# hzxie/Stereo-3D-Reconstruction

Measured on NVIDIA B200. Metric: stereo pairs/sec Stereo2Voxel fwd, higher is better.
Workload: dtype bf16

## Files before the change

### include/s3d.h

```cpp
#ifndef S3D_H_
#define S3D_H_

#include <stdint.h>

#ifdef __cplusplus
extern "C" {
#endif

#define S3D_OK                0
#define S3D_ERR_INVALID      -1
#define S3D_ERR_CUDA         -2
#define S3D_ERR_UNSUPPORTED  -3

#define S3D_DTYPE_F32   0
#define S3D_DTYPE_BF16  1
#define S3D_DTYPE_BF16X2 2

#define S3D_ACT_NONE     0
#define S3D_ACT_RELU     1
#define S3D_ACT_LEAKY    2
#define S3D_ACT_SIGMOID  3
#define S3D_ACT_TANH     4

#define S3D_MAX_TAPS 64

typedef struct S3dConvParams {
  int32_t N, iD, iH, iW, Cin;
  int32_t oD, oH, oW, Cout;
  int32_t sz, sy, sx;
  int32_t ntaps, n_classes;
  int8_t  dz[S3D_MAX_TAPS], dy[S3D_MAX_TAPS], dx[S3D_MAX_TAPS];
  int64_t osN, osD, osH, osW;
  int64_t osC;
  int64_t os_lo;
  int32_t omz, omy, omx;
  int32_t cout_store;
  int32_t in_dtype, out_dtype;
  int32_t act;  float act_param;
  int32_t tw, th, td, tn;
  int32_t bn;
  const float* proj_w;
  int32_t proj_channel, proj_act;
  const void* w_nstack;
  int32_t dz_nref, dz_c, dz_e, dz_pairs;
  const int32_t* dz_sched;
  long long* dz_planes;
} S3dConvParams;

const char* s3d_version(void);
const char* s3d_last_error(void);
int s3d_device_check(int dev);
int s3d_set_knob(const char* name, int value);
int s3d_get_knob(const char* name);

int s3d_conv_igemm(const S3dConvParams* p, const void* in, const void* w, const float* bias,
                   const void* residual, void* out, void* stream);
int s3d_conv_direct(const S3dConvParams* p, const void* in, const void* w, const float* bias,
                    const void* residual, void* out, void* stream);

int s3d_conv2d_halo(const void* in, const void* w, const float* bias, const void* residual, void* out, int nimg, int h, int wd,
                    int cin, int cout, int64_t osN, int64_t osH, int64_t osW, int relu, void* stream);

int s3d_pack_image(const float* img, const float* disp, float disp_scale, void* out,
                   int B, int H, int W, int Cpad, int out_dtype, void* stream);

int s3d_pack_image_u8(const uint8_t* img, const float* disp, float disp_scale, float img_scale, void* out,
                      int B, int H, int W, int Cpad, int out_dtype, void* stream);

int s3d_conv_first(const void* img, int img_u8, const float* disp, float disp_scale, const void* w, const float* bias,
                   void* out, int B, int H, int W, int cin, int cin_pad, int cout_pad, int dtype, int act,
                   float act_param, void* stream);

int s3d_conv_concat_volume(const S3dConvParams* p, const void* feat, int feat_pitch, int feat_pad, const float* bias,
                           void* out, void* stream);
int s3d_conv_concat_volume_ro(const S3dConvParams* p, const void* feat, int feat_pitch, int feat_pad, const void* w_refonce,
                              const float* bias, void* out, void* stream);
int s3d_concat_gonce_assemble(const float* maps_l, const float* maps_r, const float* edge_l, const float* edge_r,
                              const float* bias, void* out, int B, int D, int h, int w, int map_w, int out_dtype, void* stream);
int s3d_map_conv(const void* in, const void* w, float* out, int nimg, int h, int in_w, int ow, int off, int ntx, int cout,
                 int dtype, void* stream);
int s3d_cost_volume_concat(const void* feat, void* vol, int B, int h, int w, int C, int D,
                           int dtype, void* stream);
int s3d_soft_argmin(const float* cost, float* disp, int N, int D, int h, int w, float sign,
                    void* stream);


int s3d_tap_gather_soft_argmin(const float* taps, float* disp, float* disp_std_q, float* cost_out, int N, int D, int h, int w,
                               int tap_stride, float sign, void* stream);
int s3d_cls_soft_argmin(const void* x, const void* w_taps, float* disp, float* disp_std_q, int N, int D, int h, int w, int C,
                        float sign, void* stream);
int64_t s3d_conv_cls_workspace_bytes(int N, int D, int h, int w);
int s3d_conv_cls_soft_argmin(const S3dConvParams* p, const void* in, const float* bias, const void* w_taps, void* workspace,
                             float* disp, float* disp_std_q, float sign, void* stream);
int s3d_corr_soft_argmin(const void* feat, float* disp, float* disp_std_q, float* cost_out, int B, int h, int w,
                         int C, int c_real, int D, int dtype, void* stream);
int s3d_upsample_disp(const float* disp_q, float* disp, int N, int h, int w, int H, int W,
                      float scale, void* stream);
int s3d_upsample_disp_eval(const float* disp_q, float* disp, int B, int h, int w, int H, int W, float scale,
                           const float* gt, const float* thresholds, int T, float max_gt, long long* disp_stats,
                           uint8_t* lr_mask, float lr_thresh, long long* lr_stats,
                           const float* disp_std_q, float* disp_std, const float* unc_thresh, int K, long long* unc_stats,
                           void* stream);

int s3d_latent_to_vox(const void* x, void* out, int N, int H, int W, int C, int L, int dtype,
                      void* stream);
int s3d_avg_pool(const void* x, void* out, int N, int H, int W, int C, int L, int dtype,
                 void* stream);
int s3d_depth_to_space(const void* in, void* out, const float* proj_w, int proj_act, int N, int d, int h, int w,
                       int Cpad, int dtype, void* stream);
int s3d_split_tf32(const float* x, float* hi, float* lo, int64_t n, void* stream);
int s3d_split_bf16(const float* x, void* out, int64_t npix, int C, void* stream);
// ... 28 lines not shown
```

### stereo_3d_reconstruction_b200/csrc/concat_gonce.cu

```cuda
#include "common.cuh"

namespace s3d {
namespace {

constexpr int kMaps = 6 * 64;
constexpr int kEdge = 4 * 64;

__device__ __forceinline__ void add8(float (&v)[8], const float* __restrict__ p) {
  const float4 a = __ldg(reinterpret_cast<const float4*>(p)), b = __ldg(reinterpret_cast<const float4*>(p) + 1);
  v[0] += a.x;  v[1] += a.y;  v[2] += a.z;  v[3] += a.w;  v[4] += b.x;  v[5] += b.y;  v[6] += b.z;  v[7] += b.w;
}

template <bool kSplit>
__global__ void __launch_bounds__(256)
gonce_assemble_kernel(const float* __restrict__ maps_l, const float* __restrict__ maps_r, const float* __restrict__ edge_l,
                      const float* __restrict__ edge_r, const float* __restrict__ bias, __nv_bfloat16* __restrict__ out,
                      int B, int D, int h, int w, int mw) {
  const int x = blockIdx.x * 32 + (threadIdx.x >> 3), co = (threadIdx.x & 7) * 8;
  const int y = blockIdx.y, n = blockIdx.z;
  if (x >= w) return;
  const bool left_ref = n < B;
  const int b = left_ref ? n : n - B;
  const float* pm = (left_ref ? maps_l : maps_r) + (((int64_t)b * h + y) * mw + (x + 2)) * kMaps + co;
  const float* gm = (left_ref ? maps_r : maps_l) + ((int64_t)b * h + y) * mw * kMaps + 3 * 64 + co;
  const bool edge = x == (left_ref ? w - 1 : 0);
  const float* em = (left_ref ? edge_r : edge_l) + ((int64_t)b * h + y) * D * kEdge + co;
  float base[8];
  {
    const float4 b0 = __ldg(reinterpret_cast<const float4*>(bias + co)), b1 = __ldg(reinterpret_cast<const float4*>(bias + co) + 1);
    base[0] = b0.x;  base[1] = b0.y;  base[2] = b0.z;  base[3] = b0.w;  base[4] = b1.x;  base[5] = b1.y;  base[6] = b1.z;  base[7] = b1.w;
    add8(base, pm);
  }
  constexpr int kCo = kSplit ? 128 : 64;
  __nv_bfloat16* op = out + ((((int64_t)n * D) * h + y) * w + x) * kCo + co;
  const int64_t plane = (int64_t)h * w * kCo;
#pragma unroll 4
  for (int d = 0; d < D; ++d) {
    float v[8];
#pragma unroll
    for (int i = 0; i < 8; ++i) v[i] = base[i];
    const int col = (left_ref ? x - d : x + d) + 2;
    const bool in = col >= 0 && col < mw;
    if (in) add8(v, gm + (int64_t)col * kMaps);
    if (d == 0)     { add8(v, pm + 64);   if (in) add8(v, gm + (int64_t)col * kMaps + 64); }
    if (d == D - 1) { add8(v, pm + 128);  if (in) add8(v, gm + (int64_t)col * kMaps + 128); }
    if (edge) {
      const float* e = em + (int64_t)(left_ref ? D - 1 - d : d) * kEdge;
      add8(v, e);
      if (d == 0) add8(v, e + 64);
      if (d == D - 1) add8(v, e + 128);
    }
    uint32_t oh[4], ol[4];
#pragma unroll
    for (int i = 0; i < 4; ++i) {
      const float a0 = fmax_nan(v[2 * i], 0.f), a1 = fmax_nan(v[2 * i + 1], 0.f);
      __nv_bfloat162 t = __floats2bfloat162_rn(a0, a1);
      oh[i] = *reinterpret_cast<uint32_t*>(&t);
      if constexpr (kSplit) {
        const float2 hf = __bfloat1622float2(t);
        __nv_bfloat162 l = __floats2bfloat162_rn(a0 - hf.x, a1 - hf.y);
        ol[i] = *reinterpret_cast<uint32_t*>(&l);
      }
    }
    const uint4 o = make_uint4(oh[0], oh[1], oh[2], oh[3]);
    __stcs(reinterpret_cast<uint4*>(op + d * plane), o);
    if constexpr (kSplit) __stcs(reinterpret_cast<uint4*>(op + d * plane + 64), make_uint4(ol[0], ol[1], ol[2], ol[3]));
  }
}

}
}

extern "C" int s3d_concat_gonce_assemble(const float* maps_l, const float* maps_r, const float* edge_l, const float* edge_r,
                                         const float* bias, void* out, int B, int D, int h, int w, int map_w, int out_dtype,
                                         void* stream) {
  using namespace s3d;
  if (!maps_l || !maps_r || !edge_l || !edge_r || !bias || !out) { set_error("concat_gonce_assemble: null argument"); return S3D_ERR_INVALID; }
  S3D_CHECK_ARG(B > 0 && D >= 2 && h > 0 && w > 0 && map_w == w + 4, "concat_gonce_assemble: B=%d D=%d h=%d w=%d map_w=%d (needs D >= 2, map_w = w + 4)", B, D, h, w, map_w);
  S3D_CHECK_ARG(((reinterpret_cast<uintptr_t>(maps_l) | reinterpret_cast<uintptr_t>(maps_r) | reinterpret_cast<uintptr_t>(edge_l) |
                  reinterpret_cast<uintptr_t>(edge_r) | reinterpret_cast<uintptr_t>(bias) | reinterpret_cast<uintptr_t>(out)) & 15) == 0,
                "concat_gonce_assemble: pointers must be 16-byte aligned");
  S3D_CHECK_ARG(h <= 65535 && 2 * B <= 65535, "concat_gonce_assemble: grid too large");
  S3D_CHECK_ARG(out_dtype == S3D_DTYPE_BF16 || out_dtype == S3D_DTYPE_BF16X2, "concat_gonce_assemble: out_dtype %d", out_dtype);
  dim3 grid(ceil_div(w, 32), h, 2 * B);
  if (out_dtype == S3D_DTYPE_BF16X2)
    gonce_assemble_kernel<true><<<grid, 256, 0, static_cast<cudaStream_t>(stream)>>>(maps_l, maps_r, edge_l, edge_r, bias,
                                                                                     static_cast<__nv_bfloat16*>(out), B, D, h, w, map_w);
  else
    gonce_assemble_kernel<false><<<grid, 256, 0, static_cast<cudaStream_t>(stream)>>>(maps_l, maps_r, edge_l, edge_r, bias,
                                                                                      static_cast<__nv_bfloat16*>(out), B, D, h, w, map_w);
  S3D_LAUNCH_CHECK();
  return S3D_OK;
}
```

### stereo_3d_reconstruction_b200/csrc/conv_scatter.cu

```cuda
#include "conv_scatter.cuh"

namespace s3d {
using namespace scatter;

bool conv_scatter_eligible(const S3dConvParams* p) {
  const int esz = p->in_dtype == S3D_DTYPE_F32 ? 4 : 2;
  const bool split = p->in_dtype == S3D_DTYPE_BF16X2;
  if (!p->w_nstack || knobs().no_scatter) return false;
  if (split && (p->out_dtype != S3D_DTYPE_BF16X2 || p->Cin > 64 || (p->Cout != 16 && p->Cout != 32 && p->Cout != 64) ||
                p->cout_store != p->Cout)) return false;
  if (!split && p->out_dtype == S3D_DTYPE_BF16X2) return false;
  if (!plane_scatter_layer(*p)) return false;
  const int cin_bytes = (split ? 2 : 1) * p->Cin * esz;
  if (split && cin_bytes == 32) return false;
  if (cin_bytes != 32 && cin_bytes != 64 && cin_bytes != 128 && cin_bytes != 256) return false;
  if (p->Cout > 64 || p->Cout % 16 != 0) return false;
  return true;
}

int conv_scatter_launch(const S3dConvParams* p_in, const void* in, const float* bias, const void* residual, void* out,
                        cudaStream_t stream) {
  const S3dConvParams& p = *p_in;
  const bool tf32 = p.in_dtype == S3D_DTYPE_F32;
  const bool split = p.in_dtype == S3D_DTYPE_BF16X2;
  const int esz = tf32 ? 4 : 2;
  const int cin_phys = split ? 2 * p.Cin : p.Cin;
  S3D_CHECK_ARG(p.cout_store >= 1 && p.cout_store <= p.Cout, "scatter: cout_store");
  ScArgs a;
  memset(&a, 0, sizeof(a));
  a.p = p;  a.bias = bias;  a.residual = residual;  a.out = out;
  a.split = split ? 1 : 0;
  a.os_lo = p.os_lo ? p.os_lo : (int64_t)p.Cout;
  const int nchunks = cin_phys * esz == 256 ? 2 : 1;
  int64_t total = plane_geometry(a, cin_phys * esz / nchunks, cin_phys / nchunks, nchunks);
  a.cp = p.Cout;
  a.tps = spec_tps(a.row_bytes, a.cp);
  if (knobs().scatter_tps3 && a.tps == 9) a.tps = 3;
  S3D_CHECK_ARG(total > 0 && total < (1ll << 31), "scatter: column count out of range");
  {
    const int sms = num_sms();
    int nz = knobs().scatter_zsplit > 0 ? knobs().scatter_zsplit : (knobs().scatter_zsplit < 0 ? 1 : (int)(sms / total));
    if (nz > p.oD / 4) nz = p.oD / 4;
    if (nz > 1) {
      a.zc = ceil_div(p.oD, nz);
      a.nz = ceil_div(p.oD, a.zc);
      a.dl = a.zc + 2;
      if (a.nz > 1) total *= a.nz; else { a.nz = 1; a.zc = p.oD; a.dl = p.oD; }
    }
  }
  int grid = num_sms();
  a.pair = ((3 * a.cp / 2) % 8 == 0 && total >= 2 && grid >= 2 && !knobs().scatter_no_pair) ? 1 : 0;
  const bool fast_ok = coalesced_store_ok(p, bias, out, residual, p.out_dtype == S3D_DTYPE_F32 ? 4 : 2) &&
                       (split || !knobs().scatter_no_transpose);
  const bool two = fast_ok && a.pair && !tf32 && !split && a.nchunks == 1 && p.out_dtype == S3D_DTYPE_BF16 && residual == nullptr &&
                   spec_kernel(a.row_bytes, a.cp, false, p.act == S3D_ACT_RELU, true) != nullptr && total > grid &&
                   !knobs().scatter_generic && !knobs().scatter_one_cta && !knobs().scatter_tps3 && !knobs().scatter_ring;
  if (two) grid *= 2;
  grid = deal_columns(a, total, grid);
  const bool dz = p.dz_nref > 0 && !tf32 && !split && a.nz == 1 && !knobs().no_dz_skip;
  if (dz) S3D_CHECK_ARG(p.N == 2 * p.dz_nref && p.dz_c >= 0 && p.dz_e >= 0, "scatter: constant-region descriptor");
  if (!dz) a.p.dz_nref = 0;
  if (!dz || !a.pair) a.p.dz_sched = nullptr;
  if (a.p.dz_sched) {
    S3D_CHECK_ARG(p.dz_pairs >= 1, "scatter: dz_pairs");
    grid = 2 * p.dz_pairs;
  }
  const int w_rows = a.pair ? 3 * a.cp / 2 : 3 * a.cp;
  a.w_tx = a.tps * w_rows * a.row_bytes;
  a.w_bytes = align1024(a.w_tx);
  const int budget = two ? 110 * 1024 : 227 * 1024 - 1024 - 512;
  int ring = (budget - 4 * a.w_bytes) / a.slot_bytes;
  if (ring > kMaxRing) ring = kMaxRing;
  if (ring < 2) ring = 2;
  if (a.row_bytes == 128 && ring > (a.pair && a.nchunks == 1 ? 3 : 2)) ring = a.pair && a.nchunks == 1 ? 3 : 2;
  if (const int r = knobs().scatter_ring) { if (r >= 2 && r <= kMaxRing) ring = r; }
  a.ring = ring;
  a.w_stages = (budget - a.ring * a.slot_bytes) / a.w_bytes;
  if (a.w_stages > kMaxW) a.w_stages = kMaxW;
  S3D_CHECK_ARG(a.w_stages >= 2, "scatter: not enough shared memory for the weight ring");
  a.idesc = ptx::make_instr_desc(tf32 ? 2 : 1, a.pair ? 256 : 128, 3 * a.cp);
  a.res_direct = !knobs().scatter_res_transpose;
  a.fast_store = fast_ok;
  if (split) {
    S3D_CHECK_ARG(a.fast_store && (a.os_lo * 2) % 16 == 0 && a.os_lo >= p.Cout,
                  "scatter (split operands): needs a bias, a none / ReLU / LeakyReLU activation and 16-byte aligned out / residual / strides");
    a.res_direct = 1;
  }

  const CUtensorMapSwizzle sw = a.row_bytes == 128 ? CU_TENSOR_MAP_SWIZZLE_128B
                              : a.row_bytes == 64 ? CU_TENSOR_MAP_SWIZZLE_64B : CU_TENSOR_MAP_SWIZZLE_32B;
  CUtensorMap map_x, map_w;
  cuuint32_t box[5] = {(cuuint32_t)a.kc, kHX, kHY, 1, 1};
// ... 8 lines not shown
                  p.osW == 64 && p.osH == (int64_t)p.oW * 64 && p.osD == (int64_t)p.oH * p.osH && p.osN == (int64_t)p.oD * p.osD &&
                  !knobs().scatter_no_rm && !knobs().scatter_generic;
  if (rm) {
    const int extra = kResBytes + 32 * 128;
    a.w_stages = (budget - a.ring * a.slot_bytes - extra) / a.w_bytes;
    if (a.w_stages > kMaxW) a.w_stages = kMaxW;
    S3D_CHECK_ARG(a.w_stages >= 3, "scatter: not enough shared memory for the residual stage");
    CUtensorMap map_r;
    cuuint32_t rbox[5] = {64, kTX, kTY, 1, 1};
    rc = encode_act_map(&map_r, residual, 2, false, 64, p.oW, p.oH, p.oD, p.N, rbox, estr, CU_TENSOR_MAP_SWIZZLE_128B);
    if (rc != S3D_OK) return rc;
    a.residual = nullptr;
    const int smem_rm = a.ring * a.slot_bytes + a.w_stages * a.w_bytes + extra + 1024;
    return launch_plane_scatter(rm_kernel(p.act == S3D_ACT_RELU), grid, smem_rm, a.pair, stream, map_x, map_w, map_r, a);
  }

  const int smem_bytes = a.ring * a.slot_bytes + a.w_stages * a.w_bytes + 1024;
  KernFn kern = a.pair ? (tf32 ? conv_scatter_kernel<true, true> : conv_scatter_kernel<false, true>)
                       : (tf32 ? conv_scatter_kernel<true, false> : conv_scatter_kernel<false, false>);
  if (split) {
    const bool lean = a.pair && a.tps == spec_tps(a.row_bytes, a.cp) && !knobs().scatter_generic;
    kern = split_kernel(lean, a.pair != 0, cin_phys * esz, a.cp, residual != nullptr, p.act == S3D_ACT_RELU);
  }
  else if (a.pair && !tf32 && a.nchunks == 1 && p.out_dtype == S3D_DTYPE_BF16 && a.fast_store && a.tps == spec_tps(a.row_bytes, a.cp) &&
      !knobs().scatter_generic) {
    const bool relu = p.act == S3D_ACT_RELU;
    if (KernFn k = spec_kernel(a.row_bytes, a.cp, residual != nullptr, relu, two && a.fast_store)) kern = k;
    else if (two) { set_error("scatter: the two-CTA kernel needs the coalesced store path"); return S3D_ERR_INVALID; }
  }
  return launch_plane_scatter(kern, grid, smem_bytes, a.pair, stream, map_x, map_w, a);
}

}
```

### stereo_3d_reconstruction_b200/layers.py

```python
import ctypes
import os
import itertools

import torch

from . import lib as _lib

PAD = 16


def pad_to(c, m=PAD):
    return (c + m - 1) // m * m


def torch_dtype(code):
    return torch.float32 if code == _lib.DTYPE_F32 else torch.bfloat16


def is_split(code):
    return code == _lib.DTYPE_BF16X2


def cmult(code):
    return 2 if code == _lib.DTYPE_BF16X2 else 1
# ... 77 lines not shown
    return xr + c + 2


def dz_jump(zs, D, e):
    ze = D - 2 - e
    return (ze - zs) // 3 * 3 if ze - zs >= 3 else 0


def dz_march(zs, J, D):
    out, p = [], 0
    while p < D:
        out.append(p)
        p = p + 1 + J if p == zs + 1 else p + 1
    return out


def dz_schedule(N, nref, oH, oW, D, c, e, npairs):
    total = scatter_columns(N, oH, oW)
    first = [dz_first(k, N, nref, oH, oW, c) for k in range(total)]
    cols = sorted(range(total), key=lambda k: (first[k], k))
    items = [(cols[i], cols[i + 1] if i + 1 < total else total) for i in range(0, total, 2)]
    cost = [D - dz_jump(max(first[a], first[b] if b < total else 0), D, e) for a, b in items]
    load, lists = [0] * npairs, [[] for _ in range(npairs)]
    for i in sorted(range(len(items)), key=lambda i: (-cost[i], i)):
        q = min(range(npairs), key=lambda q: (load[q], q))
        load[q] += cost[i]
        lists[q].append(items[i])
    offs, ent = [0], []
    for lst in lists:
        offs.append(offs[-1] + len(lst))
        for a, b in lst:
            ent += [a, b]
    return offs + ent, load


class PackedConv:

    def __init__(self, w_rows, bias, taps, stride, out_mult, cin, cout, act, act_param, dtype_code, device,
                 ksize=(1, 1, 1), pad=(0, 0, 0)):
        self._ctor = (w_rows.detach().float().cpu(), bias.detach().float().cpu(), taps, stride, out_mult, cin,
                      cout, act, act_param, dtype_code, device, tuple(ksize), tuple(pad))
        self.n_classes = len(taps)
        self.ntaps = len(taps[0])
        assert self.n_classes * self.ntaps <= _lib.S3D_MAX_TAPS
        self.cin, self.cout = cin, cout
        self.cin_pad, self.cout_pad = pad_to(cin), pad_to(cout)
        self.stride = stride
        self.out_mult = out_mult
        self.act, self.act_param = act, float(act_param)
        self.dtype_code = dtype_code
        wp = torch.zeros(self.n_classes * self.ntaps, self.cout_pad, self.cin_pad, dtype=torch.float32)
        wp[:, :cout, :cin] = w_rows.cpu()
        self.weight = to_storage(wp, dtype_code).to(device).contiguous()
        bp = torch.zeros(self.cout_pad, dtype=torch.float32)
        bp[:cout] = bias.cpu()
        self.bias = bp.to(device)
        self.taps = taps
        self.ksize, self.pad = tuple(ksize), tuple(pad)
        self.weight_ns = None
        if tuple(ksize) == (3, 3, 3) and tuple(pad) == (1, 1, 1) and tuple(stride) == (1, 1, 1) and \
                self.n_classes == 1 and self.cout_pad <= 64:
            w3 = wp.view(3, 9, self.cout_pad, self.cin_pad)
            self.weight_ns = to_storage(self.pack_nstack(w3), dtype_code).to(device).contiguous()
        self.bn = _choose_bn(self.cout_pad)
        self.proj = None
        self._cache = {}
# ... 358 lines not shown
```

### stereo_3d_reconstruction_b200/lib.py

```python
import ctypes
import os

_HERE = os.path.dirname(os.path.abspath(__file__))
LIB_PATH = os.environ.get('S3D_LIB_PATH') or os.path.join(_HERE, 'libs3d_b200.so')

S3D_MAX_TAPS = 64
DTYPE_F32, DTYPE_BF16, DTYPE_BF16X2 = 0, 1, 2
ACT_NONE, ACT_RELU, ACT_LEAKY, ACT_SIGMOID, ACT_TANH = 0, 1, 2, 3, 4


class S3dConvParams(ctypes.Structure):
    _fields_ = [
        ('N', ctypes.c_int32), ('iD', ctypes.c_int32), ('iH', ctypes.c_int32), ('iW', ctypes.c_int32),
        ('Cin', ctypes.c_int32),
        ('oD', ctypes.c_int32), ('oH', ctypes.c_int32), ('oW', ctypes.c_int32), ('Cout', ctypes.c_int32),
        ('sz', ctypes.c_int32), ('sy', ctypes.c_int32), ('sx', ctypes.c_int32),
        ('ntaps', ctypes.c_int32), ('n_classes', ctypes.c_int32),
        ('dz', ctypes.c_int8 * S3D_MAX_TAPS), ('dy', ctypes.c_int8 * S3D_MAX_TAPS),
        ('dx', ctypes.c_int8 * S3D_MAX_TAPS),
        ('osN', ctypes.c_int64), ('osD', ctypes.c_int64), ('osH', ctypes.c_int64), ('osW', ctypes.c_int64),
        ('osC', ctypes.c_int64),
        ('os_lo', ctypes.c_int64),
        ('omz', ctypes.c_int32), ('omy', ctypes.c_int32), ('omx', ctypes.c_int32),
        ('cout_store', ctypes.c_int32),
        ('in_dtype', ctypes.c_int32), ('out_dtype', ctypes.c_int32),
        ('act', ctypes.c_int32), ('act_param', ctypes.c_float),
        ('tw', ctypes.c_int32), ('th', ctypes.c_int32), ('td', ctypes.c_int32), ('tn', ctypes.c_int32),
        ('bn', ctypes.c_int32),
        ('proj_w', ctypes.c_void_p), ('proj_channel', ctypes.c_int32), ('proj_act', ctypes.c_int32),
        ('w_nstack', ctypes.c_void_p),
        ('dz_nref', ctypes.c_int32), ('dz_c', ctypes.c_int32), ('dz_e', ctypes.c_int32), ('dz_pairs', ctypes.c_int32),
        ('dz_sched', ctypes.c_void_p), ('dz_planes', ctypes.c_void_p),
    ]


_vp, _i, _f, _i64 = ctypes.c_void_p, ctypes.c_int, ctypes.c_float, ctypes.c_int64
_CONV_SIG = [ctypes.POINTER(S3dConvParams), _vp, _vp, _vp, _vp, _vp, _vp]

SIGNATURES = {
    's3d_version': ([], ctypes.c_char_p),
    's3d_last_error': ([], ctypes.c_char_p),
    's3d_device_check': ([_i], _i),
    's3d_set_knob': ([ctypes.c_char_p, _i], _i),
    's3d_get_knob': ([ctypes.c_char_p], _i),
    's3d_conv_igemm': (_CONV_SIG, _i),
    's3d_conv_direct': (_CONV_SIG, _i),
    's3d_pack_image': ([_vp, _vp, _f, _vp, _i, _i, _i, _i, _i, _vp], _i),
    's3d_pack_image_u8': ([_vp, _vp, _f, _f, _vp, _i, _i, _i, _i, _i, _vp], _i),
    's3d_conv_first': ([_vp, _i, _vp, _f, _vp, _vp, _vp, _i, _i, _i, _i, _i, _i, _i, _i, _f, _vp], _i),
    's3d_conv_concat_volume': ([ctypes.POINTER(S3dConvParams), _vp, _i, _i, _vp, _vp, _vp], _i),
    's3d_conv_concat_volume_ro': ([ctypes.POINTER(S3dConvParams), _vp, _i, _i, _vp, _vp, _vp, _vp], _i),
    's3d_conv_cls_workspace_bytes': ([_i, _i, _i, _i], ctypes.c_int64),
    's3d_conv_cls_soft_argmin': ([ctypes.POINTER(S3dConvParams), _vp, _vp, _vp, _vp, _vp, _vp, ctypes.c_float, _vp], _i),
    's3d_conv2d_halo': ([_vp, _vp, _vp, _vp, _vp, _i, _i, _i, _i, _i, _i64, _i64, _i64, _i, _vp], _i),
    's3d_map_conv': ([_vp, _vp, _vp, _i, _i, _i, _i, _i, _i, _i, _i, _vp], _i),
    's3d_concat_gonce_assemble': ([_vp, _vp, _vp, _vp, _vp, _vp, _i, _i, _i, _i, _i, _i, _vp], _i),
    's3d_cost_volume_concat': ([_vp, _vp, _i, _i, _i, _i, _i, _i, _vp], _i),
    's3d_soft_argmin': ([_vp, _vp, _i, _i, _i, _i, _f, _vp], _i),
    's3d_tap_gather_soft_argmin': ([_vp, _vp, _vp, _vp, _i, _i, _i, _i, _i, _f, _vp], _i),
    's3d_cls_soft_argmin': ([_vp, _vp, _vp, _vp, _i, _i, _i, _i, _i, _f, _vp], _i),
    's3d_corr_soft_argmin': ([_vp, _vp, _vp, _vp, _i, _i, _i, _i, _i, _i, _i, _vp], _i),
    's3d_upsample_disp': ([_vp, _vp, _i, _i, _i, _i, _i, _f, _vp], _i),
    's3d_upsample_disp_eval': ([_vp, _vp, _i, _i, _i, _i, _i, _f,
                                _vp, ctypes.POINTER(_f), _i, _f, _vp,
                                _vp, _f, _vp,
                                _vp, _vp, ctypes.POINTER(_f), _i, _vp, _vp], _i),
    's3d_latent_to_vox': ([_vp, _vp, _i, _i, _i, _i, _i, _i, _vp], _i),
    's3d_avg_pool': ([_vp, _vp, _i, _i, _i, _i, _i, _i, _vp], _i),
    's3d_depth_to_space': ([_vp, _vp, _vp, _i, _i, _i, _i, _i, _i, _i, _vp], _i),
    's3d_split_tf32': ([_vp, _vp, _vp, _i64, _vp], _i),
    's3d_split_bf16': ([_vp, _vp, _i64, _i, _vp], _i),
    's3d_unsplit_bf16': ([_vp, _vp, _i64, _i, _vp], _i),
    's3d_fuse_views': ([_vp, _i64, _vp, _i64, _i, _vp, _i, _i, _i, _vp, ctypes.POINTER(_f), _i, _vp, _i64, _i64, _vp], _i),
    's3d_voxel_surface_workspace_bytes': ([_i, _i, _i], ctypes.c_int64),
    's3d_voxel_surface_eval': ([_vp, _vp, _i, _i, ctypes.POINTER(_f), _i, ctypes.POINTER(_i), _i, _vp, _vp, _i64, _vp], _i),
    's3d_voxel_mesh_bounds': ([_i, ctypes.POINTER(_i), ctypes.POINTER(_i)], _i),
    's3d_voxel_mesh': ([_vp, _i, _i, _f, _vp, _i, _vp, _i, _vp, _vp], _i),
    's3d_chamfer_forward': ([_vp, _vp, _vp, _vp, _vp, _vp, _i, _i, _i, _vp], _i),
    's3d_chamfer_workspace_bytes': ([_i, _i, _i], ctypes.c_int64),
    's3d_chamfer_forward_ws': ([_vp, _vp, _vp, _vp, _vp, _vp, _i, _i, _i, _vp, _i64, _vp], _i),
    's3d_chamfer_eval': ([_vp, _vp, _vp, _vp, _vp, _vp, _i, _i, _i, ctypes.POINTER(_f), _i, _vp, _vp, _i64, _vp], _i),
    's3d_fma_probe': ([_vp, _i, ctypes.POINTER(ctypes.c_int64), _vp], _i),
}

_lib = None


class S3dError(RuntimeError):
    pass
# ... 53 lines not shown
```

### stereo_3d_reconstruction_b200/models.py

```python
import collections
import ctypes
import math
import os

import torch
import torch.nn as nn

from . import lib as _lib
from . import ops
from .layers import PackedConv, SplitConv, pad_to, torch_dtype, cmult, more_columns_than_pairs

A = _lib

PRECISIONS = ('bf16', 'bf16x3', 'tf32', 'tf32x3', 'fp32')

OPTIONAL_OUTPUTS = (('disp_gt', ('disp_stats',)),
                    ('lr_check', ('lr_mask', 'lr_stats')),
                    ('uncertainty', ('disp_std', 'unc_stats')),
                    ('surface', ('surf_stats',)),
                    ('mesh', ('mesh_verts', 'mesh_faces', 'mesh_counts')))
_VOXEL_ONLY = {'surface': 'surface=True evaluates voxel surfaces: Stereo2Voxel only',
               'mesh': 'mesh=True meshes the voxel occupancy: Stereo2Voxel only'}

Options = collections.namedtuple('Options', 'gt disp_gt lr_check uncertainty surface mesh')
# ... 194 lines not shown
        P['enc5'] = PackedConv.from_conv(e.conv5, None, A.ACT_NONE, dc, dev)
        if self.cfg.NETWORK.COST_VOLUME == 'concat':
            ag = self.dispnet.aggregation
            for n in ('dres0a', 'dres0b', 'dres1a', 'dres1b', 'cls_a'):
                seq = getattr(ag, n)
                P[n] = PackedConv.from_conv(seq[0], seq[1], A.ACT_NONE if n == 'dres1b' else A.ACT_RELU, dc, dev)
            wb = ag.cls_b.weight
            P['cls_b'] = PackedConv.from_pointwise(wb[0].reshape(wb.shape[1], 27).t(), None, None, A.ACT_NONE, dc, dev)
        for i, seq in enumerate(self.rgbd_encoder.layers):
            P['rec%d' % i] = PackedConv.from_conv(seq[0], seq[1], A.ACT_RELU, dc, dev)
        self._pack_head(P, dc, dev)
        if self.precision == 'tf32x3':
            P = {k: SplitConv(v) for k, v in P.items()}
        self._packed = P
        self._packed_prec = self.precision
        self._ws = {}
        self._graphs = {}
        return self

    def _pack_head(self, P, dc, dev):
        raise NotImplementedError

    def _buf(self, name, shape, dtype, zero=False):
        key = (name, tuple(shape), dtype)
        t = self._ws.get(key)
        if t is None:
            dev = next(self.parameters()).device
            t = (torch.zeros if zero else torch.empty)(shape, dtype=dtype, device=dev)
            self._ws[key] = t
        return t

    def _conv(self, name, x, **kw):
        return self._packed[name](x, engine=self._engine(), **kw)

    @staticmethod
    def _bhw(img):
        return (img.shape[0], img.shape[1], img.shape[2]) if img.dtype == torch.uint8 else (img.shape[0], img.shape[2], img.shape[3])

    def _disparity(self, left, right, disp_gt=None, lr_check=False, uncertainty=False):
        cfg = self.cfg
        B, H, W = self._bhw(left)
        D = cfg.NETWORK.MAX_DISP
        dt = torch_dtype(self._dtype_code())
        x = self._first('enc0', 'e0', 'img', left, right, None, 1.0)
        x = self._conv('enc1', x, out=self._bufo('e1', 'enc1', x))
        x = self._conv('enc2', x, out=self._bufo('e2', 'enc2', x))
        y = self._conv('enc3', x, out=self._bufo('e3', 'enc3', x))
        x = self._conv('enc4', y, residual=x, out=self._bufo('e4', 'enc4', y))
        h, w = x.shape[2], x.shape[3]
        C = cfg.NETWORK.FEAT_CHANNELS
        p5, p0 = self._packed['enc5'], self._packed.get('dres0a')
        ro_split = (self._split and C == 32 and isinstance(p0, PackedConv) and p0.cout_pad == 64 and p0.act == _lib.ACT_RELU and
                    not _lib.KNOBS['no_ref_once'])
        sheared = (cfg.NETWORK.COST_VOLUME == 'concat' and (self.precision == 'bf16' or ro_split) and C == 32 and p5.cout_pad == C and
                   isinstance(p0, PackedConv) and p0.weight_ns is not None and p0.cout_pad == 64 and p0.act == _lib.ACT_RELU and
                   D >= 4 and w + 2 <= 127 and not _lib.KNOBS['no_sheared'] and not _lib.KNOBS['no_concat_fuse'] and
                   not _lib.KNOBS['no_scatter'])
        fuse_volume = (cfg.NETWORK.COST_VOLUME == 'concat' and (self.precision in ('bf16', 'tf32') or ro_split) and p5.cout_pad == C and
                       isinstance(p0, PackedConv) and p0.weight_ns is not None and
                       (ro_split or C * x.element_size() in (32, 64)) and
                       not _lib.KNOBS['no_concat_fuse'] and not _lib.KNOBS['no_scatter'] and
                       (sheared or more_columns_than_pairs(2 * B, h, w)))
        cm = cmult(self._dtype_code())
        if fuse_volume:
            pad, P = D, w + 2 * D
            Cp = cm * C
            featp = self._buf('featp', (2 * B, 1, h, P, Cp), dt, zero=True)
            self._conv('enc5', x, out=featp, out_view=(pad * Cp, (h * P * Cp, h * P * Cp, P * Cp, Cp), C if self._split else 0),
                       cout_store=C)
            feat = None
        else:
            feat = self._conv('enc5', x, out=self._bufo('e5', 'enc5', x))
        disp_q = self._buf('disp_q', (2 * B, h, w), torch.float32)
        std_q = self._buf('disp_std_q', (2 * B, h, w), torch.float32) if uncertainty else None
        std_kw = {} if std_q is None else {'std_out': std_q}
        if cfg.NETWORK.COST_VOLUME == 'concat':
            if fuse_volume:
                ro = ro_split or (self.precision == 'bf16' and p0.cout_pad == 64 and p0.act == _lib.ACT_RELU and
                                  not _lib.KNOBS['no_ref_once'])
                if sheared:
                    bufs = {'maps_l': self._buf('sh_ml', (B, 1, h, w + 4, 384), torch.float32),
                            'maps_r': self._buf('sh_mr', (B, 1, h, w + 4, 384), torch.float32),
                            'edge_l': self._buf('sh_el', (B, 1, h, D, 256), torch.float32),
                            'edge_r': self._buf('sh_er', (B, 1, h, D, 256), torch.float32)}
                    a = ops.conv_concat_volume_sheared(p0, featp, B, D, pad, out=self._buf('a0', (2 * B, D, h, w, cm * 64), dt), bufs=bufs)
                else:
                    a = ops.conv_concat_volume(p0, featp, B, D, pad, out=self._buf('a0', (2 * B, D, h, w, cm * p0.cout_pad), dt),
                                               ref_once=ro)
            else:
                assert feat.shape[-1] == cm * C, 'FEAT_CHANNELS must be a multiple of 16'
                vol = ops.cost_volume_concat(feat, B, D, out=self._buf('vol', (2 * B, D, h, w, 2 * cm * C), dt), split=self._split)
                a = self._conv('dres0a', vol, out=self._bufo('a0', 'dres0a', vol))
            bf = self.precision == 'bf16'
            a = self._conv('dres0b', a, out=self._bufo('a1', 'dres0b', a), dz=(B, 3, 1) if bf else None)
            y = self._conv('dres1a', a, out=self._bufo('a2', 'dres1a', a), dz=(B, 5, 2) if bf else None)
            a = self._conv('dres1b', y, residual=a, out=self._bufo('a3', 'dres1b', y), dz=(B, 7, 3) if bf else None)
            S = self._packed['cls_b'].cout_pad
            pa = self._packed['cls_a']
            if (self.precision == 'bf16' and isinstance(pa, PackedConv) and pa.weight_ns is not None and pa.cin_pad == 64 and
                    pa.cout_pad == 64 and pa.act == _lib.ACT_RELU and S == 32 and a.shape[-1] == 64 and
                    more_columns_than_pairs(2 * B, h, w) and
                    not _lib.KNOBS['no_cls_chain'] and not _lib.KNOBS['no_cls_fused'] and not _lib.KNOBS['no_scatter']):
                nb = ops.conv_cls_workspace_bytes(2 * B, D, h, w)
                ops.conv_cls_soft_argmin(pa, a, self._packed['cls_b'].weight, -1.0, out=disp_q,
                                         workspace=self._buf('cls_ws', (nb,), torch.uint8), **std_kw)
                return self._upsample_disp(disp_q, H, W, disp_gt, lr_check, std_q)
            c = self._conv('cls_a', a, out=self._bufo('a0', 'cls_a', a))
            if self.precision == 'bf16' and c.shape[-1] in (16, 32, 64) and S == 32 and not _lib.KNOBS['no_cls_fused']:
                ops.cls_soft_argmin(c, self._packed['cls_b'].weight, -1.0, out=disp_q, **std_kw)
            else:
                taps = self._buf('taps', (2 * B, D, h, S, w), torch.float32)
                self._conv('cls_b', c, out=taps, out_view=(0, (D * h * S * w, h * S * w, S * w, 1, w)), cout_store=S)
                ops.tap_gather_soft_argmin(taps, -1.0, out=disp_q, **std_kw)
        else:
            if self._split:
                feat = ops.unsplit_bf16(feat, out=self._buf('feat32', feat.shape[:-1] + (feat.shape[-1] // 2,), torch.float32))
            ops.corr_soft_argmin(feat, B, D, out=disp_q, c_real=C, **std_kw)
        return self._upsample_disp(disp_q, H, W, disp_gt, lr_check, std_q)
# ... 372 lines not shown
```

### stereo_3d_reconstruction_b200/ops.py

```python
import ctypes
import math

import torch

from . import lib as _lib


def _code(t):
    if t.dtype == torch.bfloat16:
        return _lib.DTYPE_BF16
    if t.dtype == torch.float32:
        return _lib.DTYPE_F32
    raise TypeError('unsupported dtype %s' % t.dtype)


def _code_like(t, split):
    if split:
        assert t.dtype == torch.bfloat16 and t.shape[-1] % 2 == 0
        return _lib.DTYPE_BF16X2
    return _code(t)


def _chk(*ts):
    for t in ts:
# ... 159 lines not shown
    _lib.count_launch()
    return out


def conv_concat_volume(pc, featp, B, D, pad, out=None, ref_once=False):
    import ctypes
    from .layers import is_split
    _chk(featp, out)
    split = is_split(pc.dtype_code)
    cm = 2 if split else 1
    n2, one, h, pitch, C = featp.shape
    C //= cm
    assert n2 == 2 * B and one == 1 and featp.is_contiguous() and pc.cin_pad == 2 * C and pad >= D - 1
    assert not split or ref_once, 'split (BF16X2) operands: reference-once form only'
    w = pitch - 2 * pad
    assert w > 0
    Co = cm * pc.cout_pad
    if out is None:
        out = torch.empty((2 * B, D, h, w, Co), dtype=featp.dtype, device=featp.device)
    assert out.is_contiguous() and out.shape == (2 * B, D, h, w, Co)
    p = pc.params(2 * B, D, h, w, (D * h * w * Co, h * w * Co, w * Co, Co), _code_like(out, split), pc.cout_pad)
    if ref_once:
        rc = _lib.load().s3d_conv_concat_volume_ro(ctypes.byref(p), featp.data_ptr(), pitch, pad, pc.refonce_weights(C).data_ptr(),
                                                   pc.bias.data_ptr(), out.data_ptr(), _stream())
        _lib.check(rc, 's3d_conv_concat_volume_ro')
    else:
        rc = _lib.load().s3d_conv_concat_volume(ctypes.byref(p), featp.data_ptr(), pitch, pad, pc.bias.data_ptr(), out.data_ptr(),
                                                _stream())
        _lib.check(rc, 's3d_conv_concat_volume')
    _lib.count_launch()
    return out


def conv_concat_volume_sheared(pc, featp, B, D, pad, out=None, bufs=None):
    from .layers import is_split
    _chk(featp, out)
    split = is_split(pc.dtype_code)
    cm = 2 if split else 1
    n2, one, h, pitch, C = featp.shape
    C //= cm
    assert n2 == 2 * B and one == 1 and featp.is_contiguous() and featp.dtype == torch.bfloat16
    assert pc.cin_pad == 2 * C and pc.cout_pad == 64 and pc.act == _lib.ACT_RELU and pad >= D - 1 and D >= 2
    w = pitch - 2 * pad
    g = pc.gonce_convs(C, pad, w, D)
    bufs = {} if bufs is None else bufs
    res = {}
    use_mc = C == 32 and not _lib.KNOBS['no_map_conv']
    for name, key, sl in (('left', 'maps_l', slice(0, B)), ('right', 'maps_r', slice(B, 2 * B)),
                          ('edge_left', 'edge_l', slice(0, B)), ('edge_right', 'edge_r', slice(B, 2 * B))):
        conv = g[name]
        off, ntx, ow = g[name + '_geom']
        o = bufs.get(key)
        if o is None:
            o = torch.empty((B, 1, h, ow, conv.cout_pad), dtype=torch.float32, device=featp.device)
        assert o.shape == (B, 1, h, ow, conv.cout_pad) and o.dtype == torch.float32 and o.is_contiguous()
        if use_mc:
            x = featp[sl]
            rc = _lib.load().s3d_map_conv(x.data_ptr(), conv.weight.data_ptr(), o.data_ptr(), B, h, pitch, ow, off, ntx,
                                          conv.cout_pad, pc.dtype_code, _stream())
            _lib.check(rc, 's3d_map_conv')
            _lib.count_launch()
            res[key] = o
        else:
            res[key] = conv(featp[sl], out=o)
    Co = cm * 64
    if out is None:
        out = torch.empty((2 * B, D, h, w, Co), dtype=torch.bfloat16, device=featp.device)
    assert out.is_contiguous() and out.shape == (2 * B, D, h, w, Co) and out.dtype == torch.bfloat16
    rc = _lib.load().s3d_concat_gonce_assemble(res['maps_l'].data_ptr(), res['maps_r'].data_ptr(), res['edge_l'].data_ptr(),
                                               res['edge_r'].data_ptr(), pc.bias.data_ptr(), out.data_ptr(), B, D, h, w, w + 4,
                                               _lib.DTYPE_BF16X2 if split else _lib.DTYPE_BF16, _stream())
    _lib.check(rc, 's3d_concat_gonce_assemble')
    _lib.count_launch()
    return out


def cls_soft_argmin(x, w_taps, sign=-1.0, out=None, std_out=None):
    _chk(x, w_taps, out)
    assert x.dtype == torch.bfloat16 and w_taps.dtype == torch.bfloat16 and x.dim() == 5 and x.is_contiguous()
    N, D, h, w, C = x.shape
    assert w_taps.numel() == 32 * C and w_taps.is_contiguous()
    if out is None:
        out = torch.empty((N, h, w), dtype=torch.float32, device=x.device)
    std = None if std_out is None else _std_buf(std_out, out).data_ptr()
    rc = _lib.load().s3d_cls_soft_argmin(x.data_ptr(), w_taps.data_ptr(), out.data_ptr(), std, N, D, h, w, C, float(sign),
                                         _stream())
    _lib.check(rc, 's3d_cls_soft_argmin')
    _lib.count_launch()
    return out


def conv_cls_workspace_bytes(N, D, h, w):
    return int(_lib.load().s3d_conv_cls_workspace_bytes(N, D, h, w))


def conv_cls_soft_argmin(pc, x, w_taps, sign=-1.0, out=None, workspace=None, std_out=None):
    import ctypes
    _chk(x, w_taps, out, workspace)
    assert x.dtype == torch.bfloat16 and w_taps.dtype == torch.bfloat16 and x.dim() == 5 and x.is_contiguous()
    N, D, h, w, C = x.shape
    assert C == 64 and pc.cin_pad == 64 and pc.cout_pad == 64 and w_taps.numel() == 32 * 64 and w_taps.is_contiguous()
    need = conv_cls_workspace_bytes(N, D, h, w)
    if workspace is None:
        workspace = torch.empty(need, dtype=torch.uint8, device=x.device)
# ... 267 lines not shown
```

Baseline: 5123.

## Skip writing cost-volume depth runs that the next conv never reads

Adds a per-column skip table of depth ranges [lo,hi) that the following dz-skipping scatter conv (dres0b) will not read, given its constant-region schedule. The gonce assemble kernel then skips storing those depth planes, which cuts write bandwidth on the large first cost volume. The table is computed on the host once per shape and cached. Correctness now depends on the Python model of the scatter walk and pairing schedule matching the kernel exactly. Stale values are left in the unread regions.

```diff
diff --git a/include/s3d.h b/include/s3d.h
--- a/include/s3d.h
+++ b/include/s3d.h
@@ -55,6 +55,10 @@
 
 int s3d_conv_igemm(const S3dConvParams* p, const void* in, const void* w, const float* bias,
                    const void* residual, void* out, void* stream);
+#define S3D_DZ_WALK_ALL   0
+#define S3D_DZ_WALK_OWN   1
+#define S3D_DZ_WALK_PAIRS 2
+int s3d_conv_dz_walk(const S3dConvParams* p);
 int s3d_conv_direct(const S3dConvParams* p, const void* in, const void* w, const float* bias,
                     const void* residual, void* out, void* stream);
 
@@ -77,6 +81,9 @@
                               const float* bias, void* out, void* stream);
 int s3d_concat_gonce_assemble(const float* maps_l, const float* maps_r, const float* edge_l, const float* edge_r,
                               const float* bias, void* out, int B, int D, int h, int w, int map_w, int out_dtype, void* stream);
+int s3d_concat_gonce_assemble_skip(const float* maps_l, const float* maps_r, const float* edge_l, const float* edge_r,
+                                   const float* bias, const int* skip, void* out, int B, int D, int h, int w, int map_w,
+                                   int out_dtype, void* stream);
 int s3d_map_conv(const void* in, const void* w, float* out, int nimg, int h, int in_w, int ow, int off, int ntx, int cout,
                  int dtype, void* stream);
 int s3d_cost_volume_concat(const void* feat, void* vol, int B, int h, int w, int C, int D,
diff --git a/stereo_3d_reconstruction_b200/csrc/concat_gonce.cu b/stereo_3d_reconstruction_b200/csrc/concat_gonce.cu
--- a/stereo_3d_reconstruction_b200/csrc/concat_gonce.cu
+++ b/stereo_3d_reconstruction_b200/csrc/concat_gonce.cu
@@ -14,8 +14,8 @@
 template <bool kSplit>
 __global__ void __launch_bounds__(256)
 gonce_assemble_kernel(const float* __restrict__ maps_l, const float* __restrict__ maps_r, const float* __restrict__ edge_l,
-                      const float* __restrict__ edge_r, const float* __restrict__ bias, __nv_bfloat16* __restrict__ out,
-                      int B, int D, int h, int w, int mw) {
+                      const float* __restrict__ edge_r, const float* __restrict__ bias, const int2* __restrict__ skip,
+                      __nv_bfloat16* __restrict__ out, int B, int D, int h, int w, int mw) {
   const int x = blockIdx.x * 32 + (threadIdx.x >> 3), co = (threadIdx.x & 7) * 8;
   const int y = blockIdx.y, n = blockIdx.z;
   if (x >= w) return;
@@ -34,8 +34,11 @@
   constexpr int kCo = kSplit ? 128 : 64;
   __nv_bfloat16* op = out + ((((int64_t)n * D) * h + y) * w + x) * kCo + co;
   const int64_t plane = (int64_t)h * w * kCo;
+  const int2 run = skip ? __ldg(skip + (int64_t)n * w + x) : make_int2(0, 0);
+  const unsigned run_len = run.y > run.x ? (unsigned)(run.y - run.x) : 0u;
 #pragma unroll 4
   for (int d = 0; d < D; ++d) {
+    if ((unsigned)(d - run.x) < run_len) continue;
     float v[8];
 #pragma unroll
     for (int i = 0; i < 8; ++i) v[i] = base[i];
@@ -71,11 +74,12 @@
 }
 }
 
-extern "C" int s3d_concat_gonce_assemble(const float* maps_l, const float* maps_r, const float* edge_l, const float* edge_r,
-                                         const float* bias, void* out, int B, int D, int h, int w, int map_w, int out_dtype,
-                                         void* stream) {
+extern "C" int s3d_concat_gonce_assemble_skip(const float* maps_l, const float* maps_r, const float* edge_l, const float* edge_r,
+                                              const float* bias, const int* skip, void* out, int B, int D, int h, int w, int map_w,
+                                              int out_dtype, void* stream) {
   using namespace s3d;
   if (!maps_l || !maps_r || !edge_l || !edge_r || !bias || !out) { set_error("concat_gonce_assemble: null argument"); return S3D_ERR_INVALID; }
+  S3D_CHECK_ARG((reinterpret_cast<uintptr_t>(skip) & 7) == 0, "concat_gonce_assemble: skip runs must be 8-byte aligned");
   S3D_CHECK_ARG(B > 0 && D >= 2 && h > 0 && w > 0 && map_w == w + 4, "concat_gonce_assemble: B=%d D=%d h=%d w=%d map_w=%d (needs D >= 2, map_w = w + 4)", B, D, h, w, map_w);
   S3D_CHECK_ARG(((reinterpret_cast<uintptr_t>(maps_l) | reinterpret_cast<uintptr_t>(maps_r) | reinterpret_cast<uintptr_t>(edge_l) |
                   reinterpret_cast<uintptr_t>(edge_r) | reinterpret_cast<uintptr_t>(bias) | reinterpret_cast<uintptr_t>(out)) & 15) == 0,
@@ -84,11 +88,17 @@
   S3D_CHECK_ARG(out_dtype == S3D_DTYPE_BF16 || out_dtype == S3D_DTYPE_BF16X2, "concat_gonce_assemble: out_dtype %d", out_dtype);
   dim3 grid(ceil_div(w, 32), h, 2 * B);
   if (out_dtype == S3D_DTYPE_BF16X2)
-    gonce_assemble_kernel<true><<<grid, 256, 0, static_cast<cudaStream_t>(stream)>>>(maps_l, maps_r, edge_l, edge_r, bias,
-                                                                                     static_cast<__nv_bfloat16*>(out), B, D, h, w, map_w);
+    gonce_assemble_kernel<true><<<grid, 256, 0, static_cast<cudaStream_t>(stream)>>>(
+        maps_l, maps_r, edge_l, edge_r, bias, reinterpret_cast<const int2*>(skip), static_cast<__nv_bfloat16*>(out), B, D, h, w, map_w);
   else
-    gonce_assemble_kernel<false><<<grid, 256, 0, static_cast<cudaStream_t>(stream)>>>(maps_l, maps_r, edge_l, edge_r, bias,
-                                                                                      static_cast<__nv_bfloat16*>(out), B, D, h, w, map_w);
+    gonce_assemble_kernel<false><<<grid, 256, 0, static_cast<cudaStream_t>(stream)>>>(
+        maps_l, maps_r, edge_l, edge_r, bias, reinterpret_cast<const int2*>(skip), static_cast<__nv_bfloat16*>(out), B, D, h, w, map_w);
   S3D_LAUNCH_CHECK();
   return S3D_OK;
 }
+
+extern "C" int s3d_concat_gonce_assemble(const float* maps_l, const float* maps_r, const float* edge_l, const float* edge_r,
+                                         const float* bias, void* out, int B, int D, int h, int w, int map_w, int out_dtype,
+                                         void* stream) {
+  return s3d_concat_gonce_assemble_skip(maps_l, maps_r, edge_l, edge_r, bias, nullptr, out, B, D, h, w, map_w, out_dtype, stream);
+}
diff --git a/stereo_3d_reconstruction_b200/csrc/conv_scatter.cu b/stereo_3d_reconstruction_b200/csrc/conv_scatter.cu
--- a/stereo_3d_reconstruction_b200/csrc/conv_scatter.cu
+++ b/stereo_3d_reconstruction_b200/csrc/conv_scatter.cu
@@ -16,6 +16,22 @@
   if (cin_bytes != 32 && cin_bytes != 64 && cin_bytes != 128 && cin_bytes != 256) return false;
   if (p->Cout > 64 || p->Cout % 16 != 0) return false;
   return true;
+}
+
+struct ScWalk { int nz, zc; bool pair, dz; };
+
+ScWalk scatter_walk(const S3dConvParams& p, int64_t total) {
+  ScWalk wk{1, p.oD, false, false};
+  const int sms = num_sms();
+  int nz = knobs().scatter_zsplit > 0 ? knobs().scatter_zsplit : (knobs().scatter_zsplit < 0 ? 1 : (int)(sms / total));
+  if (nz > p.oD / 4) nz = p.oD / 4;
+  if (nz > 1) {
+    const int zc = ceil_div(p.oD, nz);
+    if (ceil_div(p.oD, zc) > 1) { wk.zc = zc;  wk.nz = ceil_div(p.oD, zc); }
+  }
+  wk.pair = (3 * p.Cout / 2) % 8 == 0 && total * wk.nz >= 2 && sms >= 2 && !knobs().scatter_no_pair;
+  wk.dz = p.dz_nref > 0 && p.in_dtype != S3D_DTYPE_F32 && p.in_dtype != S3D_DTYPE_BF16X2 && wk.nz == 1 && !knobs().no_dz_skip;
+  return wk;
 }
 
 int conv_scatter_launch(const S3dConvParams* p_in, const void* in, const float* bias, const void* residual, void* out,
@@ -37,19 +53,13 @@
   a.tps = spec_tps(a.row_bytes, a.cp);
   if (knobs().scatter_tps3 && a.tps == 9) a.tps = 3;
   S3D_CHECK_ARG(total > 0 && total < (1ll << 31), "scatter: column count out of range");
-  {
-    const int sms = num_sms();
-    int nz = knobs().scatter_zsplit > 0 ? knobs().scatter_zsplit : (knobs().scatter_zsplit < 0 ? 1 : (int)(sms / total));
-    if (nz > p.oD / 4) nz = p.oD / 4;
-    if (nz > 1) {
-      a.zc = ceil_div(p.oD, nz);
-      a.nz = ceil_div(p.oD, a.zc);
-      a.dl = a.zc + 2;
-      if (a.nz > 1) total *= a.nz; else { a.nz = 1; a.zc = p.oD; a.dl = p.oD; }
-    }
+  const ScWalk wk = scatter_walk(p, total);
+  if (wk.nz > 1) {
+    a.nz = wk.nz;  a.zc = wk.zc;  a.dl = wk.zc + 2;
+    total *= wk.nz;
   }
   int grid = num_sms();
-  a.pair = ((3 * a.cp / 2) % 8 == 0 && total >= 2 && grid >= 2 && !knobs().scatter_no_pair) ? 1 : 0;
+  a.pair = wk.pair ? 1 : 0;
   const bool fast_ok = coalesced_store_ok(p, bias, out, residual, p.out_dtype == S3D_DTYPE_F32 ? 4 : 2) &&
                        (split || !knobs().scatter_no_transpose);
   const bool two = fast_ok && a.pair && !tf32 && !split && a.nchunks == 1 && p.out_dtype == S3D_DTYPE_BF16 && residual == nullptr &&
@@ -57,7 +67,7 @@
                    !knobs().scatter_generic && !knobs().scatter_one_cta && !knobs().scatter_tps3 && !knobs().scatter_ring;
   if (two) grid *= 2;
   grid = deal_columns(a, total, grid);
-  const bool dz = p.dz_nref > 0 && !tf32 && !split && a.nz == 1 && !knobs().no_dz_skip;
+  const bool dz = wk.dz;
   if (dz) S3D_CHECK_ARG(p.N == 2 * p.dz_nref && p.dz_c >= 0 && p.dz_e >= 0, "scatter: constant-region descriptor");
   if (!dz) a.p.dz_nref = 0;
   if (!dz || !a.pair) a.p.dz_sched = nullptr;
@@ -132,3 +142,13 @@
 }
 
 }
+
+extern "C" int s3d_conv_dz_walk(const S3dConvParams* p) {
+  using namespace s3d;
+  if (!p) { set_error("s3d_conv_dz_walk: null argument"); return S3D_ERR_INVALID; }
+  if (!conv_scatter_eligible(p)) return S3D_DZ_WALK_ALL;
+  const ScWalk wk = scatter_walk(*p, (int64_t)p->N * ceil_div(p->oW, kTX) * ceil_div(p->oH, kTY));
+  if (!wk.dz) return S3D_DZ_WALK_ALL;
+  if (!wk.pair) return S3D_DZ_WALK_OWN;
+  return p->dz_sched ? S3D_DZ_WALK_PAIRS : S3D_DZ_WALK_ALL;
+}
diff --git a/stereo_3d_reconstruction_b200/layers.py b/stereo_3d_reconstruction_b200/layers.py
--- a/stereo_3d_reconstruction_b200/layers.py
+++ b/stereo_3d_reconstruction_b200/layers.py
@@ -133,6 +133,29 @@
         for a, b in lst:
             ent += [a, b]
     return offs + ent, load
+
+
+def dz_unread_runs(N, nref, oH, oW, D, c, e, npairs=None):
+    total = scatter_columns(N, oH, oW)
+    first = [dz_first(k, N, nref, oH, oW, c) for k in range(total)]
+    zs = list(first)
+    if npairs is not None:
+        table, _ = dz_schedule(N, nref, oH, oW, D, c, e, npairs)
+        ent = table[npairs + 1:]
+        for a, b in zip(ent[0::2], ent[1::2]):
+            zs[a] = max(first[a], first[b] if b < total else 0)
+            if b < total:
+                zs[b] = zs[a]
+    cy, cx = -(-oH // 32), -(-oW // 8)
+    runs = [[(0, D)] * oW for _ in range(N)]
+    for k in range(total):
+        n, x0 = k // (cy * cx), (k % cx) * 8
+        lo = zs[k] + 2
+        hi = lo + dz_jump(zs[k], D, e)
+        for x in range(max(0, x0 - 1), min(oW, x0 + 9)):
+            a, b = runs[n][x]
+            runs[n][x] = (max(a, lo), min(b, hi))
+    return [[(a, b) if b > a else (0, 0) for a, b in row] for row in runs]
 
 
 class PackedConv:
diff --git a/stereo_3d_reconstruction_b200/lib.py b/stereo_3d_reconstruction_b200/lib.py
--- a/stereo_3d_reconstruction_b200/lib.py
+++ b/stereo_3d_reconstruction_b200/lib.py
@@ -7,6 +7,7 @@
 S3D_MAX_TAPS = 64
 DTYPE_F32, DTYPE_BF16, DTYPE_BF16X2 = 0, 1, 2
 ACT_NONE, ACT_RELU, ACT_LEAKY, ACT_SIGMOID, ACT_TANH = 0, 1, 2, 3, 4
+DZ_WALK_ALL, DZ_WALK_OWN, DZ_WALK_PAIRS = 0, 1, 2
 
 
 class S3dConvParams(ctypes.Structure):
@@ -55,6 +56,8 @@
     's3d_conv2d_halo': ([_vp, _vp, _vp, _vp, _vp, _i, _i, _i, _i, _i, _i64, _i64, _i64, _i, _vp], _i),
     's3d_map_conv': ([_vp, _vp, _vp, _i, _i, _i, _i, _i, _i, _i, _i, _vp], _i),
     's3d_concat_gonce_assemble': ([_vp, _vp, _vp, _vp, _vp, _vp, _i, _i, _i, _i, _i, _i, _vp], _i),
+    's3d_conv_dz_walk': ([_vp], _i),
+    's3d_concat_gonce_assemble_skip': ([_vp, _vp, _vp, _vp, _vp, _vp, _vp, _i, _i, _i, _i, _i, _i, _vp], _i),
     's3d_cost_volume_concat': ([_vp, _vp, _i, _i, _i, _i, _i, _i, _vp], _i),
     's3d_soft_argmin': ([_vp, _vp, _i, _i, _i, _i, _f, _vp], _i),
     's3d_tap_gather_soft_argmin': ([_vp, _vp, _vp, _vp, _i, _i, _i, _i, _i, _f, _vp], _i),
diff --git a/stereo_3d_reconstruction_b200/models.py b/stereo_3d_reconstruction_b200/models.py
--- a/stereo_3d_reconstruction_b200/models.py
+++ b/stereo_3d_reconstruction_b200/models.py
@@ -250,6 +250,23 @@
 
     def _conv(self, name, x, **kw):
         return self._packed[name](x, engine=self._engine(), **kw)
+
+    def _a0_skip(self, B, D, h, w):
+        pb = self._packed['dres0b']
+        p = pb.params(2 * B, D, h, w, (D * h * w * 64, h * w * 64, w * 64, 64), _lib.DTYPE_BF16, 64, 0, (B, 3, 1))
+        walk = _lib.load().s3d_conv_dz_walk(ctypes.byref(p))
+        if walk < 0:
+            _lib.check(walk, 's3d_conv_dz_walk')
+        if walk == _lib.DZ_WALK_ALL:
+            return None
+        key = ('a0_skip', B, D, h, w, walk)
+        t = self._ws.get(key)
+        if t is None:
+            from .layers import dz_unread_runs
+            runs = dz_unread_runs(2 * B, B, h, w, D, 3, 1, p.dz_pairs if walk == _lib.DZ_WALK_PAIRS else None)
+            t = torch.tensor(runs, dtype=torch.int32).to(next(self.parameters()).device)
+            self._ws[key] = t
+        return t
 
     @staticmethod
     def _bhw(img):
@@ -301,7 +318,8 @@
                             'maps_r': self._buf('sh_mr', (B, 1, h, w + 4, 384), torch.float32),
                             'edge_l': self._buf('sh_el', (B, 1, h, D, 256), torch.float32),
                             'edge_r': self._buf('sh_er', (B, 1, h, D, 256), torch.float32)}
-                    a = ops.conv_concat_volume_sheared(p0, featp, B, D, pad, out=self._buf('a0', (2 * B, D, h, w, cm * 64), dt), bufs=bufs)
+                    a = ops.conv_concat_volume_sheared(p0, featp, B, D, pad, out=self._buf('a0', (2 * B, D, h, w, cm * 64), dt), bufs=bufs,
+                                                       skip=self._a0_skip(B, D, h, w) if self.precision == 'bf16' else None)
                 else:
                     a = ops.conv_concat_volume(p0, featp, B, D, pad, out=self._buf('a0', (2 * B, D, h, w, cm * p0.cout_pad), dt),
                                                ref_once=ro)
diff --git a/stereo_3d_reconstruction_b200/ops.py b/stereo_3d_reconstruction_b200/ops.py
--- a/stereo_3d_reconstruction_b200/ops.py
+++ b/stereo_3d_reconstruction_b200/ops.py
@@ -215,7 +215,7 @@
     return out
 
 
-def conv_concat_volume_sheared(pc, featp, B, D, pad, out=None, bufs=None):
+def conv_concat_volume_sheared(pc, featp, B, D, pad, out=None, bufs=None, skip=None):
     from .layers import is_split
     _chk(featp, out)
     split = is_split(pc.dtype_code)
@@ -250,9 +250,13 @@
     if out is None:
         out = torch.empty((2 * B, D, h, w, Co), dtype=torch.bfloat16, device=featp.device)
     assert out.is_contiguous() and out.shape == (2 * B, D, h, w, Co) and out.dtype == torch.bfloat16
-    rc = _lib.load().s3d_concat_gonce_assemble(res['maps_l'].data_ptr(), res['maps_r'].data_ptr(), res['edge_l'].data_ptr(),
-                                               res['edge_r'].data_ptr(), pc.bias.data_ptr(), out.data_ptr(), B, D, h, w, w + 4,
-                                               _lib.DTYPE_BF16X2 if split else _lib.DTYPE_BF16, _stream())
+    maps = (res['maps_l'].data_ptr(), res['maps_r'].data_ptr(), res['edge_l'].data_ptr(), res['edge_r'].data_ptr(), pc.bias.data_ptr())
+    odt = _lib.DTYPE_BF16X2 if split else _lib.DTYPE_BF16
+    if skip is None:
+        rc = _lib.load().s3d_concat_gonce_assemble(*maps, out.data_ptr(), B, D, h, w, w + 4, odt, _stream())
+    else:
+        assert skip.dtype == torch.int32 and skip.is_cuda and skip.is_contiguous() and skip.shape == (2 * B, w, 2)
+        rc = _lib.load().s3d_concat_gonce_assemble_skip(*maps, skip.data_ptr(), out.data_ptr(), B, D, h, w, w + 4, odt, _stream())
     _lib.check(rc, 's3d_concat_gonce_assemble')
     _lib.count_launch()
     return out
```

New measurement: 5114 (median of 6 runs). About the same (-0.2%).
